# Bitcoin-Wildlife-Sanctuary/recursive-stwo

Hardware: AMD Instinct MI355X
Metric: recursive proofs verified/sec (higher is better)
Workload: dtype u32 (M31 modular integers)

## Files before the change

### recursive-stwo_amd/csrc/field.hpp

```cpp
#pragma once
#include <hip/hip_runtime.h>
#include <stdint.h>

namespace rsv {

constexpr uint32_t P = 0x7fffffffu;

__device__ __forceinline__ uint32_t m_add(uint32_t a, uint32_t b) {
    uint32_t s = a + b;
    return min(s, s - P);
}
__device__ __forceinline__ uint32_t m_sub(uint32_t a, uint32_t b) {
    uint32_t d = a - b;
    return min(d, d + P);
}
__device__ __forceinline__ uint32_t m_neg(uint32_t a) { return m_sub(0u, a); }
__device__ __forceinline__ uint32_t m_dbl(uint32_t a) { return m_add(a, a); }
__device__ __forceinline__ uint32_t m_mul(uint32_t a, uint32_t b) {
    uint64_t p = (uint64_t)a * b;
    uint32_t s = ((uint32_t)p & P) + (uint32_t)(p >> 31);
    return min(s, s - P);
}
__device__ __forceinline__ uint32_t m_sqr(uint32_t a) { return m_mul(a, a); }
__device__ __forceinline__ uint32_t m_shl(uint32_t a, uint32_t k) {
    return ((a << k) & P) | (a >> (31u - k));
}
__device__ inline uint32_t m_inv(uint32_t a) {
    uint32_t t1 = a;
    uint32_t t2 = m_mul(m_sqr(t1), t1);
    uint32_t t4 = t2;
    for (int i = 0; i < 2; i++) t4 = m_sqr(t4);
    t4 = m_mul(t4, t2);
    uint32_t t8 = t4;
    for (int i = 0; i < 4; i++) t8 = m_sqr(t8);
    t8 = m_mul(t8, t4);
    uint32_t t16 = t8;
    for (int i = 0; i < 8; i++) t16 = m_sqr(t16);
    t16 = m_mul(t16, t8);
    uint32_t t24 = t16;
    for (int i = 0; i < 8; i++) t24 = m_sqr(t24);
    t24 = m_mul(t24, t8);
    uint32_t t28 = t24;
    for (int i = 0; i < 4; i++) t28 = m_sqr(t28);
    t28 = m_mul(t28, t4);
    uint32_t t29 = m_mul(m_sqr(t28), t1);
    return m_mul(m_sqr(m_sqr(t29)), t1);
}

struct CM31 {
    uint32_t a, b;
};
struct QM31 {
    CM31 a, b;
};

__device__ __forceinline__ CM31 c_mk(uint32_t a, uint32_t b) { return CM31{a, b}; }
__device__ __forceinline__ CM31 c_add(CM31 x, CM31 y) { return {m_add(x.a, y.a), m_add(x.b, y.b)}; }
__device__ __forceinline__ CM31 c_sub(CM31 x, CM31 y) { return {m_sub(x.a, y.a), m_sub(x.b, y.b)}; }
__device__ __forceinline__ CM31 c_neg(CM31 x) { return {m_neg(x.a), m_neg(x.b)}; }
__device__ __forceinline__ CM31 c_mul(CM31 x, CM31 y) {
    return {m_sub(m_mul(x.a, y.a), m_mul(x.b, y.b)), m_add(m_mul(x.a, y.b), m_mul(x.b, y.a))};
}
__device__ __forceinline__ CM31 c_mul_m(CM31 x, uint32_t k) { return {m_mul(x.a, k), m_mul(x.b, k)}; }
__device__ __forceinline__ CM31 c_mul_r(CM31 x) {
    return {m_sub(m_dbl(x.a), x.b), m_add(m_dbl(x.b), x.a)};
}
__device__ inline CM31 c_inv(CM31 x) {
    uint32_t n = m_inv(m_add(m_sqr(x.a), m_sqr(x.b)));
    return {m_mul(x.a, n), m_mul(m_neg(x.b), n)};
}

__device__ __forceinline__ QM31 q_mk(uint32_t a0, uint32_t a1, uint32_t b0, uint32_t b1) {
    return QM31{{a0, a1}, {b0, b1}};
}
__device__ __forceinline__ QM31 q_zero() { return q_mk(0, 0, 0, 0); }
__device__ __forceinline__ QM31 q_one() { return q_mk(1, 0, 0, 0); }
__device__ __forceinline__ QM31 q_from_m(uint32_t x) { return q_mk(x, 0, 0, 0); }
__device__ __forceinline__ QM31 q_add(QM31 x, QM31 y) { return {c_add(x.a, y.a), c_add(x.b, y.b)}; }
__device__ __forceinline__ QM31 q_sub(QM31 x, QM31 y) { return {c_sub(x.a, y.a), c_sub(x.b, y.b)}; }
__device__ __forceinline__ QM31 q_neg(QM31 x) { return {c_neg(x.a), c_neg(x.b)}; }
__device__ __forceinline__ QM31 q_dbl(QM31 x) { return q_add(x, x); }
__device__ __forceinline__ QM31 q_mul(QM31 x, QM31 y) {
    CM31 ac = c_mul(x.a, y.a), bd = c_mul(x.b, y.b);
    return {c_add(ac, c_mul_r(bd)), c_add(c_mul(x.a, y.b), c_mul(x.b, y.a))};
}
__device__ __forceinline__ QM31 q_mul_m(QM31 x, uint32_t k) { return {c_mul_m(x.a, k), c_mul_m(x.b, k)}; }
__device__ __forceinline__ QM31 q_mul_c(QM31 x, CM31 k) { return {c_mul(x.a, k), c_mul(x.b, k)}; }
__device__ inline QM31 q_inv(QM31 x) {
    CM31 den = c_inv(c_sub(c_mul(x.a, x.a), c_mul_r(c_mul(x.b, x.b))));
    return {c_mul(x.a, den), c_mul(c_neg(x.b), den)};
}
__device__ __forceinline__ bool q_eq(QM31 x, QM31 y) {
    return ((x.a.a ^ y.a.a) | (x.a.b ^ y.a.b) | (x.b.a ^ y.b.a) | (x.b.b ^ y.b.b)) == 0;
}
__device__ __forceinline__ QM31 q_mul_i(QM31 x) { return q_mk(m_neg(x.a.b), x.a.a, m_neg(x.b.b), x.b.a); }
__device__ __forceinline__ QM31 q_mul_u(QM31 x) { return {c_mul_r(x.b), x.a}; }
__device__ __forceinline__ QM31 q_combine_ef(QM31 v0, QM31 v1, QM31 v2, QM31 v3) {
    return q_add(q_add(v0, q_mul_i(v1)), q_add(q_mul_u(v2), q_mul_u(q_mul_i(v3))));
}

}
```

### recursive-stwo_amd/csrc/k_plan.hpp

```cpp
#pragma once
#include "verify_common.hpp"

namespace rsv {

struct PlanPtrs {
    PlanHdr* hdr;
    uint32_t* ent;
    uint32_t* fl;
    uint32_t G, maxM;
    const uint32_t* ids;
    uint32_t p0;
    __device__ uint32_t proof_of(uint32_t slot) const { return ids ? ids[slot] : p0 + slot; }
};

constexpr int MAX_FUSED = 16;
template <class Args>
struct Fused {
    uint32_t nb;
    uint32_t lds_proofs;
    uint32_t first_block[MAX_FUSED + 1];
    uint8_t y_of[32];
    Args a[MAX_FUSED];
};
constexpr size_t plan_lds_bytes(uint32_t proofs) { return (size_t)proofs * (32 * 2 * 8 + 3 * 32 * 4); }
// ... 189 lines not shown
    const bool live = livep && j < nq;
    ProofCtx* c = livep ? &ctxs[p] : nullptr;
    const uint32_t gbase = grp * G;
    for (uint32_t i = threadIdx.x; i < pb * 32u * 2u; i += BLOCK) (&F[0][0][0])[i] = 0ull;
    const uint32_t v0 = live ? (c->raw_q[j] & ((1u << M) - 1u)) : 0xFFFFFFFFu;
    raw[threadIdx.x] = v0;
    __syncthreads();
    if (live) {
        uint32_t rank = 0;
        for (uint32_t k = 0; k < nq; k++) {
            const uint32_t vk = raw[gbase + k];
            rank += (vk < v0 || (vk == v0 && k < j)) ? 1u : 0u;
        }
        sq[gbase + rank] = v0;
        sp[gbase + rank] = (uint8_t)j;
    }
    __syncthreads();
    uint32_t flags = 0;
    const uint32_t v = live ? sq[gbase + j] : 0u;
    if (live) {
        c->q[j] = v;
        c->qperm[j] = sp[gbase + j];
        if (j + 1 < nq && sq[gbase + j + 1] == v) flags |= 1u << R_DUP_QUERY;
        uint32_t lstart = 0;
        if (j > 0) {
            const uint32_t x = v ^ sq[gbase + j - 1];
            lstart = x ? M - (31u - (uint32_t)__clz((int)x)) : M + 1u;
        }
        for (uint32_t l = lstart; l <= M; l++) atomicOr(&F[grp][l][j >> 6], 1ull << (j & 63u));
    }
    __syncthreads();
    auto mask = [&](uint32_t l) { return M128{F[grp][l][0], F[grp][l][1]}; };
    uint32_t sizes[3] = {M, A == B ? A : umax(A, B), A == B ? 0u : umin(A, B)};
    const uint32_t n_sizes = A == B ? 2u : 3u;
    auto is_size = [&](uint32_t l) { return l == sizes[0] || l == sizes[1] || (n_sizes == 3 && l == sizes[2]); };
    if (live) {
        for (uint32_t l = j; l <= M; l += nq) {
            const M128 Fl = mask(l);
            const uint32_t nodes = m128_pop(Fl);
            uint32_t lacking = 0;
            if (l >= 1) lacking = 2u * m128_pop(mask(l - 1)) - nodes;
            tl[grp][l] = nodes | (lacking << 8);
            if (l < M) {
                const uint32_t both_total = m128_pop(m128_andn(mask(l + 1), Fl));
                const uint32_t nosib_total = l == 0 ? 1u : m128_pop(mask(l - 1)) - m128_pop(m128_andn(Fl, mask(l - 1)));
                tw[grp][l] = (is_size(l + 1) ? 0u : nodes - both_total) + (is_size(l) ? 2u * nosib_total : 0u);
            }
        }
    }
    __syncthreads();
    PlanHdr* h = livep ? &pl.hdr[slot] : nullptr;
    if (live && j == 0) {
        uint32_t suffix = 0;
        h->lvl[M + 1] = 0;
        for (uint32_t l = M; l >= 1; l--) {
            suffix += (tl[grp][l] >> 8) & 0xFFu;
            h->lvl[l] = tl[grp][l] | (suffix << 16);
        }
        h->lvl[0] = 1u | (suffix << 16);
        uint32_t W = 0;
        for (uint32_t l = M; l-- > 0;) {
            wsum[grp][l] = W;
            h->wf[l + 1] = (uint16_t)W;
            W += tw[grp][l];
        }
        h->wf[0] = (uint16_t)W;
        h->wf_total = (uint16_t)umin(W, 0xFFFFu);
        c->n_sizes = n_sizes;
        c->sizes[0] = sizes[0]; c->sizes[1] = sizes[1]; c->sizes[2] = n_sizes == 3 ? sizes[2] : 0u;
        uint32_t base = 0;
        for (uint32_t g = 0; g < n_sizes; g++) {
            c->fw_base[g] = base;
            base += (tl[grp][sizes[g]] >> 8) & 0xFFu;
        }
        if (base != m->first.wit_n) flags |= (1u << R_FRI_FIRST) | F_RESCAN;
    }
    __syncthreads();
    if (live) {
        uint32_t* ent = pl.ent + (size_t)slot * (pl.maxM + 1) * G;
        uint32_t* fl = pl.fl + (size_t)slot * 2 * G;
        ent[j] = 0xFFu << 16;
        for (uint32_t l = 1; l <= M; l++) {
            const M128 Fl = mask(l), Fp = mask(l - 1);
            const uint32_t s = m128_last_le(Fp, j);
            const uint32_t e = m128_first_gt(Fp, j, nq) - 1u;
            const uint32_t Ns = m128_popbelow(Fl, s + 1), Ne = m128_popbelow(Fl, e + 1), Nj = m128_popbelow(Fl, j + 1);
            const bool both = Ne - Ns == 1u;
            const bool right = both && Nj - Ns == 1u;
            const uint32_t second = both ? m128_first_gt(Fl, s, nq) : 0u;
            const uint32_t sib = both ? (right ? second - 1u : second) : 0xFFu;
            const uint32_t lack_before = 2u * m128_popbelow(Fp, s) - m128_popbelow(Fl, s);
            ent[l * G + j] = (Nj - 1u) | (lack_before << 8) | (sib << 16);
        }
        for (uint32_t d = 0; d + 1 < n_sizes; d++) {
            const uint32_t l = sizes[1 + d];
            if (l >= M) continue;
            const M128 Fl = mask(l), Fc = mask(l + 1);
            const uint32_t f = m128_last_le(Fl, j), e = m128_first_gt(Fl, j, nq) - 1u;
            const bool has_both = m128_popbelow(Fc, e + 1) - m128_popbelow(Fc, f + 1) == 1u;
            const bool child_data = is_size(l + 1);
            const bool lack = !child_data && !has_both;
            bool sib_present = false;
            uint32_t nosib_before = 0;
            if (l >= 1) {
                const M128 Fp = mask(l - 1);
                const uint32_t s = m128_last_le(Fp, j), pe = m128_first_gt(Fp, j, nq) - 1u;
                sib_present = m128_popbelow(Fl, pe + 1) - m128_popbelow(Fl, s + 1) == 1u;
                nosib_before = m128_popbelow(Fp, s) - m128_popbelow(m128_andn(Fl, Fp), s);
            }
            const uint32_t nodes_before = m128_popbelow(Fl, f), both_before = m128_popbelow(m128_andn(Fc, Fl), f);
            const uint32_t base = wsum[grp][l] + (child_data ? 0u : nodes_before - both_before) + 2u * nosib_before;
            const bool odd = (v >> (M - l)) & 1u;
            uint32_t w_self = 0xFFFFu, w_sib = 0xFFFFu;
            if (odd) {
                if (!sib_present) w_sib = base;
                if (lack) w_self = base + (sib_present ? 0u : 2u);
            } else {
                if (lack) w_self = base;
                if (!sib_present) w_sib = base + (lack ? 1u : 0u);
            }
            fl[d * G + j] = (w_self & 0xFFFFu) | (w_sib << 16);
        }
    }
    if (flags) atomicOr(&c->flags, flags);
}

constexpr uint32_t TR_WORDS = 40 + 4 * (MAX_INNER + 1) + MAXQ;
__global__ __launch_bounds__(256) void k_export_transcript(uint32_t n, const ProofMeta* __restrict__ metas,
                                                            const ProofCtx* __restrict__ ctxs, uint32_t* __restrict__ out) {
    const size_t gid = (size_t)blockIdx.x * blockDim.x + threadIdx.x;
    if (gid >= (size_t)n * TR_WORDS) return;
    const uint32_t p = (uint32_t)(gid / TR_WORDS), k = (uint32_t)(gid % TR_WORDS);
    const ProofMeta& m = metas[p];
    const ProofCtx& c = ctxs[p];
    uint32_t v = 0;
    if (m.reason != R_OK || (c.flags & (1u << R_PARSE))) v = k == 0 ? (uint32_t)R_PARSE : 0u;
    else if (k == 0) v = (c.flags & (1u << R_POW)) ? (uint32_t)R_POW : (uint32_t)R_OK;
    else if (k == 1) v = m.n_inner + 1;
    else if (k == 2) v = m.nq;
    else if (k == 3) v = m.M;
    else if (k < 8) v = c.z[k - 4];
    else if (k < 12) v = c.alpha[k - 8];
    else if (k < 16) v = c.rc[k - 12];
    else if (k < 20) v = c.oods_t[k - 16];
    else if (k < 24) v = c.oods_x[k - 20];
    else if (k < 28) v = c.oods_y[k - 24];
    else if (k < 32) v = c.after[k - 28];
    else if (k < 40) v = c.pow_digest[k - 32];
    else if (k < 40 + 4 * (MAX_INNER + 1)) { uint32_t a = (k - 40) >> 2; v = a <= m.n_inner ? c.fri_alpha[a][(k - 40) & 3] : 0u; }
    else { uint32_t q = k - (40 + 4 * (MAX_INNER + 1)); v = q < m.nq ? c.raw_q[q] : 0u; }
    out[gid] = v;
}

__global__ __launch_bounds__(64) void k_qconst(const uint8_t* __restrict__ blob, const uint64_t* __restrict__ offsets,
                                               uint32_t n, const ProofMeta* __restrict__ metas,
                                               ProofCtx* __restrict__ ctxs) {
    const uint32_t p = blockIdx.x * blockDim.x + threadIdx.x;
    if (p >= n) return;
    const ProofMeta& m = metas[p];
    if (m.reason != R_OK) return;
    ProofCtx& c = ctxs[p];
    const uint32_t* w = reinterpret_cast<const uint32_t*>(blob + offsets[p]);
    const uint32_t M = m.M, A = m.A, B = m.B;
    uint32_t sizes[3] = {M, A == B ? A : umax(A, B), A == B ? 0u : umin(A, B)};
    const uint32_t n_sizes = A == B ? 2u : 3u;
    QM31 after = ldq(c.after);
    {
        QM31 ak = q_mk(0, 0, m_neg(2), 0);
#pragma unroll 1
        for (int k = 0; k < N_APOW; k++) { stq(c.apow[k], ak); ak = q_mul(ak, after); }
    }
    QM31 ox = ldq(c.oods_x), oy = ldq(c.oods_y);
    for (uint32_t g = 0; g < n_sizes; g++) {
        uint32_t l = sizes[g];
        uint32_t comp_log = (l == A) ? m.lp : m.lq;
        CPoint step = cp_gen_mul(1u << (31u - comp_log));
        step.y = m_neg(step.y);
        QM31 sx = q_sub(q_mul_m(ox, step.x), q_mul_m(oy, step.y));
        QM31 sy = q_add(q_mul_m(ox, step.y), q_mul_m(oy, step.x));
        uint32_t k_run = 0, n_batches = (l == M) ? 1u : 2u;
        for (uint32_t bi = 0; bi < n_batches; bi++) {
            QM31 px = bi ? sx : ox, py = bi ? sy : oy;
            QM31 sa = q_zero(), sb = q_zero();
            for (int t = 0; t < 4; t++) {
                uint32_t c0, c1;
                if (l == M) { if (t != 3) continue; c0 = 0; c1 = 8; }
                else {
                    if (t == 3) continue;
                    c0 = (l == A) ? 0u : plonk_cols(t);
                    c1 = (l == B) ? tree_cols(t) : plonk_cols(t);
                }
                for (uint32_t col = c0; col < c1; col++) {
                    uint32_t ns = n_samples_of(t, (int)col);
                    if (bi == 1 && ns != 2) continue;
                    int si = sample_index(t, (int)col, bi == 1 ? 0 : (int)ns - 1);
                    QM31 v = ldq(w + SAMPLES.off[si]);
                    QM31 ak = ldq(c.apow[k_run++]);
                    sa = q_add(sa, q_mul_c(ak, v.b));
                    sb = q_add(sb, q_mul_c(ak, c_sub(c_mul(v.a, py.b), c_mul(v.b, py.a))));
                }
            }
            QBatch& qb = c.batch[g][bi];
            stq(qb.sa, sa); stq(qb.sb, sb);
            qb.prx[0] = px.a.a; qb.prx[1] = px.a.b; qb.pix[0] = px.b.a; qb.pix[1] = px.b.b;
            qb.pry[0] = py.a.a; qb.pry[1] = py.a.b; qb.piy[0] = py.b.a; qb.piy[1] = py.b.b;
        }
        c.n_batches[g] = n_batches;
    }
}

__host__ __device__ constexpr int sample_index_c(int t, int col, int s) {
    return t == 0 ? S_T0 + col : t == 1 ? S_T1 + col : t == 3 ? S_T3 + col
         : S_T2 + (col < 4 ? col : col < 8 ? 4 + 2 * (col - 4) + s : col < 12 ? 12 + (col - 8) : 16 + 2 * (col - 12) + s);
}
struct QTab {
    uint16_t n[4];
    uint8_t si[4][N_APOW];
    uint8_t batch[4][N_APOW];
};
__host__ __device__ constexpr QTab make_qtab() {
    QTab q{};
    for (int kind = 0; kind < 4; kind++) {
        int k = 0;
        const int n_batches = kind == 0 ? 1 : 2;
        for (int bi = 0; bi < n_batches; bi++)
            for (int t = 0; t < 4; t++) {
                int c0 = 0, c1 = 0;
                if (kind == 0) { if (t != 3) continue; c0 = 0; c1 = 8; }
                else {
                    if (t == 3) continue;
                    c0 = (kind == 1 || kind == 3) ? 0 : (int)plonk_cols(t);
                    c1 = (kind == 2 || kind == 3) ? (int)tree_cols(t) : (int)plonk_cols(t);
                }
                for (int col = c0; col < c1; col++) {
                    const int ns = (int)n_samples_of(t, col);
                    if (bi == 1 && ns != 2) continue;
                    q.si[kind][k] = (uint8_t)sample_index_c(t, col, bi == 1 ? 0 : ns - 1);
                    q.batch[kind][k] = (uint8_t)bi;
                    k++;
                }
            }
        q.n[kind] = (uint16_t)k;
    }
    return q;
}
__constant__ QTab QTAB = make_qtab();
static_assert(make_qtab().n[3] <= N_APOW && make_qtab().n[3] == 134 && make_qtab().n[0] == 8, "alpha powers kept for the quotient numerators");

__global__ __launch_bounds__(256) void k_qconst_row(const uint8_t* __restrict__ blob, const uint64_t* __restrict__ offsets,
                                                    uint32_t n, const ProofMeta* __restrict__ metas,
                                                    ProofCtx* __restrict__ ctxs) {
    qconst_row_body(blockIdx.x, blob, offsets, n & 0x7FFFFFFFu, metas, ctxs, (n >> 31) != 0u);
}
__device__ void qconst_row_body(uint32_t block, const uint8_t* __restrict__ blob, const uint64_t* __restrict__ offsets, uint32_t n,
                                const ProofMeta* __restrict__ metas, ProofCtx* __restrict__ ctxs, bool four) {
    const uint32_t i = threadIdx.x & 15u, row = four ? (threadIdx.x >> 4) & 3u : 0u;
    const uint32_t p = (block * blockDim.x + threadIdx.x) >> (four ? 6 : 4);
    if (p >= n) return;
    const ProofMeta& m = metas[p];
    if (m.reason != R_OK) return;
    ProofCtx& c = ctxs[p];
    const uint32_t* w = reinterpret_cast<const uint32_t*>(blob + offsets[p]);
    const uint32_t M = m.M, A = m.A, B = m.B;
    const uint32_t sizes[3] = {M, A == B ? A : umax(A, B), A == B ? 0u : umin(A, B)};
    const uint32_t n_sizes = A == B ? 2u : 3u;
    auto sel = [](bool cnd, QM31 a, QM31 b) {
        return q_mk(cnd ? a.a.a : b.a.a, cnd ? a.a.b : b.a.b, cnd ? a.b.a : b.b.a, cnd ? a.b.b : b.b.b);
    };
    auto sum16 = [](QM31 x) { return q_mk(sum_row(x.a.a), sum_row(x.a.b), sum_row(x.b.a), sum_row(x.b.b)); };
    const QM31 after = ldq(c.after), one = q_one();
    const QM31 a2 = q_mul(after, after), a4 = q_mul(a2, a2), a8 = q_mul(a4, a4), a16 = q_mul(a8, a8);
    QM31 start = sel(i & 1u, after, one);
    start = q_mul(start, sel(i & 2u, a2, one));
    start = q_mul(start, sel(i & 4u, a4, one));
    start = q_mul(start, sel(i & 8u, a8, one));
    start = q_mul(start, q_mk(0, 0, m_neg(2), 0));
    if (!four || row == 3u) {
        QM31 cur = start;
#pragma unroll 1
        for (uint32_t k = i; k < (uint32_t)N_APOW; k += 16u) { stq(c.apow[k], cur); cur = q_mul(cur, a16); }
        if (four) return;
    }
    if (four && row >= n_sizes) return;
    const QM31 ox = ldq(c.oods_x), oy = ldq(c.oods_y);
    for (uint32_t g = four ? row : 0u; g < (four ? row + 1u : n_sizes); g++) {
        const uint32_t l = sizes[g];
        const uint32_t kind = l == M ? 0u : (A == B ? 3u : (l == A ? 1u : 2u));
        const uint32_t comp_log = (l == A) ? m.lp : m.lq;
        CPoint step = {GEN_POW.x[31u - comp_log], GEN_POW.y[31u - comp_log]};
        step.y = m_neg(step.y);
        const QM31 sx = q_sub(q_mul_m(ox, step.x), q_mul_m(oy, step.y));
        const QM31 sy = q_add(q_mul_m(ox, step.y), q_mul_m(oy, step.x));
        QM31 sa0 = q_zero(), sb0 = q_zero(), sa1 = q_zero(), sb1 = q_zero(), cur = start;
        const uint32_t cnt = QTAB.n[kind];
#pragma unroll 1
        for (uint32_t k0 = 0; k0 < cnt; k0 += 16u) {
            const uint32_t k = k0 + i;
            if (k < cnt) {
                const bool b1 = QTAB.batch[kind][k] != 0;
                const QM31 v = ldq(w + SAMPLES.off[QTAB.si[kind][k]]);
                const QM31 py = b1 ? sy : oy;
                const QM31 ta = q_mul_c(cur, v.b);
                const QM31 tb = q_mul_c(cur, c_sub(c_mul(v.a, py.b), c_mul(v.b, py.a)));
                sa0 = sel(b1, sa0, q_add(sa0, ta)); sb0 = sel(b1, sb0, q_add(sb0, tb));
                sa1 = sel(b1, q_add(sa1, ta), sa1); sb1 = sel(b1, q_add(sb1, tb), sb1);
            }
            cur = q_mul(cur, a16);
        }
        sa0 = sum16(sa0); sb0 = sum16(sb0); sa1 = sum16(sa1); sb1 = sum16(sb1);
        if (i == 0) {
            const uint32_t n_batches = (l == M) ? 1u : 2u;
            for (uint32_t bi = 0; bi < n_batches; bi++) {
                QBatch& qb = c.batch[g][bi];
                const QM31 px = bi ? sx : ox, py = bi ? sy : oy;
                stq(qb.sa, bi ? sa1 : sa0); stq(qb.sb, bi ? sb1 : sb0);
                qb.prx[0] = px.a.a; qb.prx[1] = px.a.b; qb.pix[0] = px.b.a; qb.pix[1] = px.b.b;
                qb.pry[0] = py.a.a; qb.pry[1] = py.a.b; qb.piy[0] = py.b.a; qb.piy[1] = py.b.b;
            }
            c.n_batches[g] = n_batches;
        }
    }
}

}
```

### recursive-stwo_amd/csrc/k_query.hpp

```cpp
#pragma once
#include "k_plan.hpp"

namespace rsv {

struct QueryArgs {
    const uint8_t* blob;
    const uint64_t* offsets;
    uint32_t n;
    const ProofMeta* metas;
    ProofCtx* ctxs;
    PlanPtrs pl;
    uint32_t* leafv;
    uint32_t maxInner;
    uint32_t* folded_out;
    uint32_t* qv_out;
    uint32_t qv_stride;
};

__device__ __forceinline__ uint32_t ent_rb(uint32_t e) { return e & 0xFFu; }
__device__ __forceinline__ uint32_t ent_lb(uint32_t e) { return (e >> 8) & 0xFFu; }
__device__ __forceinline__ uint32_t ent_sib(uint32_t e) { return (e >> 16) & 0xFFu; }
__device__ __forceinline__ uint32_t lvl_nd(uint32_t v) { return v & 0xFFu; }
__device__ __forceinline__ uint32_t lvl_tl(uint32_t v) { return (v >> 8) & 0xFFu; }
__device__ __forceinline__ uint32_t lvl_s(uint32_t v) { return v >> 16; }

__device__ inline QM31 fold_pair(QM31 self, QM31 sib, bool odd, uint32_t inv_coord, QM31 alpha) {
    QM31 l = odd ? sib : self, r = odd ? self : sib;
    return q_add(q_add(l, r), q_mul(q_mul_m(q_sub(l, r), inv_coord), alpha));
}

__device__ __forceinline__ QM31 line_eval(const uint32_t* __restrict__ cf, uint32_t log_n, uint32_t n, uint32_t x, uint32_t hi0 = 0,
                                          uint32_t hi_step = 1) {
    uint32_t r[16];
#pragma unroll
    for (int j = 0; j < 16; j++) { r[15 - j] = x; x = m_sub(m_dbl(m_sqr(x)), 1u); }
    const uint32_t s = (16u - log_n) & 15u;
#pragma unroll
    for (int st = 8; st >= 1; st >>= 1) {
        const bool on = (s & (uint32_t)st) != 0;
#pragma unroll
        for (int t = 0; t < 16; t++) {
            const uint32_t from = t + st < 16 ? r[t + st] : 1u;
            r[t] = on ? from : r[t];
        }
    }
    const uint32_t nlo = log_n < 4 ? log_n : 4u;
    uint32_t wl[16];
#pragma unroll
    for (int t = 0; t < 16; t++) wl[t] = 1u;
#pragma unroll
    for (int b = 0; b < 4; b++) {
        const uint32_t db = (uint32_t)b < nlo ? r[b] : 1u;
#pragma unroll
        for (int t = 0; t < 16; t++)
            if (t & (1 << b)) wl[t] = m_mul(wl[t], db);
    }
    QM31 acc = q_zero();
    const uint32_t n_hi = n >> nlo, n_lo = 1u << nlo;
#pragma unroll 1
    for (uint32_t hi = hi0; hi < n_hi; hi += hi_step) {
        uint32_t wh = 1u;
#pragma unroll
        for (int b = 0; b < 12; b++)
            if ((uint32_t)b + 4u < log_n && ((hi >> b) & 1u)) wh = m_mul(wh, r[b + 4]);
        QM31 inner = q_zero();
#pragma unroll
        for (int t = 0; t < 16; t++) {
            if ((uint32_t)t < n_lo) inner = q_add(inner, q_mul_m(ldq(cf + 4 * ((hi << nlo) + t)), wl[t]));
            if ((t & 3) == 3) __builtin_amdgcn_sched_barrier(0);
        }
        acc = q_add(acc, q_mul_m(inner, wh));
    }
    return acc;
}

__device__ __forceinline__ bool last_layer_ok(QM31 eval, QM31 folded) { return q_eq(eval, folded); }

template <int BLOCK, uint32_t QB, bool ROW = false>
__global__ __launch_bounds__(BLOCK) void k_query(Fused<QueryArgs> f) {
    constexpr int VB = ROW ? BLOCK / 16 : BLOCK;
    const uint32_t tid = ROW ? threadIdx.x >> 4 : threadIdx.x;
    const uint32_t part = ROW ? threadIdx.x & 15u : 0u;
    auto row_sum_q = [](QM31 v) { return q_mk(sum_row(v.a.a), sum_row(v.a.b), sum_row(v.b.a), sum_row(v.b.b)); };
    __shared__ uint32_t xq[VB][4];
    __shared__ uint32_t fst[3][4][VB];
    __shared__ uint32_t dps[3][2][VB];
    __builtin_amdgcn_s_setprio(3);
    RSV_FUSED_SELECT(f, a, bx);
    const uint32_t G = a.pl.G, per_block = VB / G;
    const uint32_t grp = tid / G, j = tid % G;
    const uint32_t slot = bx * per_block + grp;
    bool live = grp < per_block && slot < a.n;
    const uint32_t p = live ? a.pl.proof_of(slot) : 0u;
    const ProofMeta* m = live ? &a.metas[p] : nullptr;
    live = live && m->reason == R_OK && j < m->nq;
    ProofCtx* c = live ? &a.ctxs[p] : nullptr;
    const uint32_t* w = live ? reinterpret_cast<const uint32_t*>(a.blob + a.offsets[p]) : nullptr;
    const uint32_t* ent = live ? a.pl.ent + (size_t)slot * (a.pl.maxM + 1) * G : nullptr;
    const PlanHdr* h = live ? &a.pl.hdr[slot] : nullptr;
    uint32_t* leafv = live ? a.leafv + ((size_t)slot * (3 + a.maxInner)) * G * 8 : nullptr;
    const uint32_t gbase = grp * G;
    uint32_t flags = 0;
    uint32_t M = live ? m->M : 0, A = live ? m->A : 0, B = live ? m->B : 0;
    uint32_t qj = live ? c->q[j] : 0;
    uint32_t* qv = (live && a.qv_out) ? a.qv_out + ((size_t)slot * G + c->qperm[j]) * a.qv_stride : nullptr;
    uint32_t n_sizes = live ? c->n_sizes : 0;
    auto put_first = [&](uint32_t g, QM31 v) {
        fst[g][0][tid] = v.a.a; fst[g][1][tid] = v.a.b; fst[g][2][tid] = v.b.a; fst[g][3][tid] = v.b.b;
    };
    auto get_first = [&](uint32_t g) { return q_mk(fst[g][0][tid], fst[g][1][tid], fst[g][2][tid], fst[g][3][tid]); };
    if (live) {
        CPoint cur = domain_point(M, qj);
        uint32_t lvl = M;
        auto descend = [&](uint32_t g) {
            const uint32_t l = g < n_sizes ? c->sizes[g] : lvl;
            while (lvl > l) {
                const uint32_t pos = qj >> (M - lvl);
                uint32_t y2 = m_dbl(m_mul(cur.x, cur.y));
                cur.x = m_sub(m_dbl(m_sqr(cur.x)), 1u);
                cur.y = ((pos ^ (pos >> 1)) & 1u) ? m_neg(y2) : y2;
                lvl--;
            }
            dps[g][0][tid] = cur.x; dps[g][1][tid] = cur.y;
        };
        descend(0); descend(1); descend(2);
    }
    for (uint32_t g = 0; g < 3; g++) {
        QM31 answer = q_zero();
        uint32_t l = 0, pos = 0;
        bool on = live && g < n_sizes;
        uint32_t dpg_y = 0;
        if (on) {
            l = c->sizes[g];
            pos = qj >> (M - l);
            QM31 r0 = q_zero(), r1 = q_zero();
            uint32_t col = 0, dbl = 0;
            const uint32_t ncols_group = (l == M) ? 8u : ((l == A ? 30u : 0u) + (l == B ? 96u : 0u));
            for (int t = 0; t < 4; t++) {
                if ((l == M) != (t == 3)) continue;
                const uint32_t mx = (t == 3) ? M : umax(A, B);
                const uint32_t nc_leaf = (t == 3) ? 8u : ((A == mx ? plonk_cols(t) : 0u) + (B == mx ? poseidon_cols(t) : 0u));
                const uint32_t* qv = w + m->qv_off[t];
                const uint32_t qv_n = m->qv_n[t];
                for (int comp = 0; comp < 2; comp++) {
                    uint32_t cl = (t == 3) ? M : (comp == 0 ? A : B);
                    if (cl != l) continue;
                    uint32_t nc = (t == 3) ? (comp == 0 ? 8u : 0u) : (comp == 0 ? plonk_cols(t) : poseidon_cols(t));
                    if (nc == 0) continue;
                    uint32_t off;
                    if (cl == mx) off = ent_rb(ent[mx * G + j]) * nc_leaf + ((comp == 1 && A == B && t != 3) ? plonk_cols(t) : 0u);
                    else off = lvl_nd(h->lvl[mx]) * nc_leaf + ent_rb(ent[cl * G + j]) * nc;
                    bool inb = off + nc <= qv_n;
                    if (!inb) flags |= 1u << (R_MERKLE_T0 + t);
                    if constexpr (ROW) {
                        for (uint32_t k = part; k < nc; k += 16u) {
                            const uint32_t v = inb ? qv[off + k] : 0u;
                            r0 = q_add(r0, q_mul_m(ldq(c->apow[col + k]), v));
                            if (t == 2 && (k & 4u)) r1 = q_add(r1, q_mul_m(ldq(c->apow[ncols_group + dbl + 4u * (k >> 3) + (k & 3u)]), v));
                        }
                        col += nc;
                        if (t == 2) dbl += 4u * (nc >> 3) + ((nc & 7u) > 4u ? (nc & 7u) - 4u : 0u);
                    } else
                    for (uint32_t k0 = 0; k0 < nc; k0 += QB) {
                        const bool twice = t == 2 && (k0 & 4);
                        uint32_t vv[QB];
                        QM31 aa[QB];
#pragma unroll
                        for (uint32_t u = 0; u < QB; u++) {
                            const bool ok = k0 + u < nc;
                            vv[u] = (ok && inb) ? qv[off + k0 + u] : 0u;
                            aa[u] = ldq(c->apow[ok ? col + u : col]);
                        }
#pragma unroll
                        for (uint32_t u = 0; u < QB; u++) r0 = q_add(r0, q_mul_m(aa[u], vv[u]));
                        if (twice) {
#pragma unroll
                            for (uint32_t u = 0; u < QB; u++) aa[u] = ldq(c->apow[ncols_group + dbl + (k0 + u < nc ? u : 0u)]);
#pragma unroll
                            for (uint32_t u = 0; u < QB; u++) r1 = q_add(r1, q_mul_m(aa[u], vv[u]));
                        }
                        const uint32_t done = nc - k0 < QB ? nc - k0 : QB;
                        col += done;
                        if (twice) dbl += done;
                    }
                }
            }
            if constexpr (ROW) { r0 = row_sum_q(r0); r1 = row_sum_q(r1); }
            const CPoint dpg = {dps[g][0][tid], dps[g][1][tid]};
            dpg_y = dpg.y;
            for (uint32_t bi = 0; bi < c->n_batches[g]; bi++) {
                const QBatch& qb = c->batch[g][bi];
                CM31 prx = c_mk(qb.prx[0], qb.prx[1]), pix = c_mk(qb.pix[0], qb.pix[1]);
                CM31 pry = c_mk(qb.pry[0], qb.pry[1]), piy = c_mk(qb.piy[0], qb.piy[1]);
                CM31 den = c_sub(c_mul(c_sub(prx, c_mk(dpg.x, 0)), piy), c_mul(c_sub(pry, c_mk(dpg.y, 0)), pix));
                const CM31 inv_den = c_inv(den);
                __builtin_amdgcn_sched_barrier(0);
                QM31 num = q_sub(q_mul_c(bi ? r1 : r0, piy), q_add(q_mul_m(ldq(qb.sa), dpg.y), ldq(qb.sb)));
                answer = q_add(answer, q_mul_c(num, inv_den));
            }
        }
        stq(xq[tid], answer);
        __syncthreads();
        if (on) {
            uint32_t e = ent[l * G + j];
            QM31 sib;
            if (ent_sib(e) != 0xFFu) sib = ldq(xq[gbase + ent_sib(e)]);
            else {
                uint32_t wi = c->fw_base[g] + ent_lb(e);
                sib = wi < m->first.wit_n ? ldq(w + m->first.wit_off + 4 * wi) : q_zero();
                if ((sib.a.a >= P) | (sib.a.b >= P) | (sib.b.a >= P) | (sib.b.b >= P)) flags |= 1u << R_PARSE;
            }
            uint32_t* lv = leafv + ((size_t)g * G + j) * 8;
            stq(lv, answer); stq(lv + 4, sib);
            uint32_t by = (pos & 1u) ? m_neg(dpg_y) : dpg_y;
            const QM31 fg = fold_pair(answer, sib, pos & 1u, m_inv(by), ldq(c->fri_alpha[M - l]));
            put_first(g, fg);
            if (a.folded_out) stq(a.folded_out + (((size_t)slot * 3 + g) * G + c->qperm[j]) * 4, fg);
            if (qv) { stq(qv + 4 * g, answer); stq(qv + 12 + 4 * g, fg); }
        }
        __syncthreads();
    }
    QM31 folded = q_zero();
    uint32_t l = M;
    uint32_t X = live ? dps[0][0][tid] : 0u;
    for (uint32_t i = 0; i < a.maxInner; i++) {
        bool on = live && i < m->n_inner;
        if (on) {
            for (uint32_t g = 0; g < n_sizes; g++)
                if (c->sizes[g] == l) {
                    QM31 al = ldq(c->fri_alpha[i]);
                    folded = q_add(q_mul(q_mul(al, al), folded), get_first(g));
                }
            l -= 1;
        }
        stq(xq[tid], folded);
        __syncthreads();
        if (on) {
            uint32_t pos = qj >> (M - l);
            uint32_t e = ent[l * G + j];
            const FriLayerRef& L = m->inner[i];
            QM31 sib;
            if (ent_sib(e) != 0xFFu) sib = ldq(xq[gbase + ent_sib(e)]);
            else {
                uint32_t wi = ent_lb(e);
                sib = wi < L.wit_n ? ldq(w + L.wit_off + 4 * wi) : q_zero();
                if ((sib.a.a >= P) | (sib.a.b >= P) | (sib.b.a >= P) | (sib.b.b >= P)) flags |= 1u << R_PARSE;
            }
            if (j == 0 && lvl_tl(h->lvl[l]) != L.wit_n) flags |= (1u << R_FRI_INNER) | F_RESCAN;
            uint32_t* lv = leafv + ((size_t)(3 + i) * G + j) * 8;
            stq(lv, folded); stq(lv + 4, sib);
            if (qv) stq(qv + 24 + 4 * i, folded);
            uint32_t xr = (i == 0) ? X : m_sub(m_dbl(m_sqr(X)), 1u);
            X = (pos & 1u) ? m_neg(xr) : xr;
            folded = fold_pair(folded, sib, pos & 1u, m_inv(X), ldq(c->fri_alpha[i + 1]));
        }
        __syncthreads();
    }
    if (live) {
        QM31 acc = line_eval(w + m->last_off, m->log_last, m->last_n, m_sub(m_dbl(m_sqr(X)), 1u), part, ROW ? 16u : 1u);
        if constexpr (ROW) acc = row_sum_q(acc);
        if (!last_layer_ok(acc, folded)) flags |= 1u << R_FRI_LAST;
        if (qv) { stq(qv + 24 + 4 * a.maxInner, folded); stq(qv + 28 + 4 * a.maxInner, acc); }
    }
    if (flags) atomicOr(&c->flags, flags);
}

__global__ __launch_bounds__(256) void k_field_op(int op, const uint32_t* __restrict__ a, const uint32_t* __restrict__ b,
                                                   uint32_t* __restrict__ out, size_t n) {
    const size_t i = (size_t)blockIdx.x * blockDim.x + threadIdx.x;
    if (i >= n) return;
    QM31 x = ldq(a + 4 * i), y = b ? ldq(b + 4 * i) : q_zero(), r = q_zero();
    switch (op) {
        case 0: r = q_add(x, y); break;
        case 1: r = q_sub(x, y); break;
        case 2: r = q_mul(x, y); break;
        case 3: r = q_inv(x); break;
        case 4: r = q_mk(m_mul(x.a.a, y.a.a), 0, 0, 0); break;
        case 5: r = q_mk(m_inv(x.a.a), 0, 0, 0); break;
        case 6: { CM31 c = c_mul(x.a, y.a); r = q_mk(c.a, c.b, 0, 0); } break;
        case 7: { CM31 c = c_inv(x.a); r = q_mk(c.a, c.b, 0, 0); } break;
        case 8: r = q_mul_i(x); break;
        case 9: r = q_mul_u(x); break;
        case 10: {
            QM31 acc = q_one(), base = x;
            for (uint32_t e = y.a.a; e; e >>= 1) { if (e & 1u) acc = q_mul(acc, base); base = q_mul(base, base); }
            r = acc;
        } break;
        default: break;
    }
    stq(out + 4 * i, r);
}

__global__ __launch_bounds__(256) void k_domain_points(uint32_t log_size, const uint32_t* __restrict__ q,
                                                        uint32_t* __restrict__ xy, size_t n) {
    const size_t i = (size_t)blockIdx.x * blockDim.x + threadIdx.x;
    if (i >= n) return;
    CPoint p = domain_point(log_size, q[i] & ((1u << log_size) - 1u));
    xy[2 * i] = p.x; xy[2 * i + 1] = p.y;
}

__global__ __launch_bounds__(256) void k_last_layer_check(const uint32_t* __restrict__ coeffs, uint32_t log_n,
                                                           const uint32_t* __restrict__ x, const uint32_t* __restrict__ folded,
                                                           uint8_t* __restrict__ ok, size_t n) {
    const size_t i = (size_t)blockIdx.x * blockDim.x + threadIdx.x;
    if (i >= n) return;
    ok[i] = last_layer_ok(line_eval(coeffs, log_n, 1u << log_n, x[i]), ldq(folded + 4 * i)) ? 1 : 0;
}

__global__ __launch_bounds__(256) void k_line_eval(const uint32_t* __restrict__ coeffs, uint32_t log_n,
                                                    const uint32_t* __restrict__ x, uint32_t* __restrict__ out, size_t n) {
    const size_t i = (size_t)blockIdx.x * blockDim.x + threadIdx.x;
    if (i >= n) return;
    stq(out + 4 * i, line_eval(coeffs, log_n, 1u << log_n, x[i]));
}

}
```

### recursive-stwo_amd/csrc/layout.hpp

```cpp
#pragma once
#include <stdint.h>

#if !defined(__HIPCC__) && !defined(__host__)
#define __host__
#define __device__
#endif

namespace rsv {

constexpr int MAXQ = 128;
constexpr int MAX_INNER = 28;
constexpr int MAX_LOG = 30;
constexpr int N_SAMPLES = 142;
constexpr int N_APOW = 136;

__host__ __device__ constexpr uint32_t plonk_cols(int t) { return t == 0 ? 10u : t == 1 ? 12u : t == 2 ? 8u : 0u; }
__host__ __device__ constexpr uint32_t poseidon_cols(int t) { return t == 0 ? 40u : t == 1 ? 48u : t == 2 ? 8u : 0u; }
__host__ __device__ constexpr uint32_t tree_cols(int t) { return t == 3 ? 8u : plonk_cols(t) + poseidon_cols(t); }
__host__ __device__ constexpr uint32_t n_samples_of(int t, int c) { return (t == 2 && (c & 4)) ? 2u : 1u; }

constexpr uint32_t W_LP = 0, W_LQ = 1, W_PLONK_SUM = 2, W_POSEIDON_SUM = 6, W_POW_BITS = 10, W_BLOWUP = 11,
                   W_LOG_LAST = 12, W_NQ = 13, W_NCOMMIT = 15, W_COMMIT0 = 17, W_NTREES = 49;

struct SampleTable {
    uint16_t off[N_SAMPLES];
    uint16_t col_prefix[134];
    uint16_t tree_prefix[4];
    uint16_t end;
    uint16_t pre_of[N_SAMPLES];
    uint8_t cnt_of[N_SAMPLES];
};
__host__ __device__ constexpr SampleTable make_sample_table() {
    SampleTable t{};
    uint32_t pos = W_NTREES + 2, k = 0, c_all = 0;
    for (int tr = 0; tr < 4; tr++) {
        t.tree_prefix[tr] = (uint16_t)pos;
        pos += 2;
        for (uint32_t c = 0; c < tree_cols(tr); c++) {
            t.col_prefix[c_all++] = (uint16_t)pos;
            t.pre_of[k] = (uint16_t)pos;
            t.cnt_of[k] = (uint8_t)n_samples_of(tr, (int)c);
            pos += 2;
            for (uint32_t s = 0; s < n_samples_of(tr, (int)c); s++) {
                t.off[k++] = (uint16_t)pos;
                pos += 4;
            }
        }
    }
    t.end = (uint16_t)pos;
    return t;
}
constexpr int S_T0 = 0, S_T1 = 50, S_T2 = 110, S_T3 = 134;

struct FriLayerRef {
    uint32_t wit_off, wit_n;
    uint32_t hash_off, hash_n;
    uint32_t commit_off;
};

struct ProofMeta {
    uint32_t reason;
    uint32_t n_words;
    uint32_t lp, lq, pow_bits, blowup, log_last, nq, n_inner, A, B, M;
    uint32_t hw_off[4], hw_n[4];
    uint32_t qv_off[4], qv_n[4];
    uint32_t nonce_off;
    FriLayerRef first;
    FriLayerRef inner[MAX_INNER];
    uint32_t last_off, last_n;
};


struct QBatch {
    uint32_t sa[4], sb[4];
    uint32_t prx[2], pix[2], pry[2], piy[2];
};

constexpr uint32_t F_RESCAN = 1u << 30;
constexpr uint32_t F_REASON_MASK = (1u << 13) - 1u;

struct ProofCtx {
    uint32_t flags;
    uint32_t flow_on;
    uint32_t front_over;
    uint32_t n_sizes;
    uint32_t sizes[3];
    uint32_t fw_base[3];
    uint32_t z[4], alpha[4], rc[4], oods_t[4], oods_x[4], oods_y[4], after[4];
    uint32_t pow_digest[8];
    uint32_t fri_alpha[MAX_INNER + 1][4];
    uint32_t raw_q[MAXQ];
    uint32_t q[MAXQ];
    uint8_t qperm[MAXQ];
    QBatch batch[3][2];
    uint32_t n_batches[3];
    uint32_t apow[N_APOW][4];
};

__host__ __device__ constexpr uint32_t flow_chunks(uint32_t n_cols) { return (n_cols + 7u) / 8u; }
__host__ __device__ constexpr uint32_t flow_transcript_len(uint32_t nq, uint32_t n_inner, uint32_t last_n) {
    return 82u + 2u * (1u + n_inner) + (last_n + 1u) / 2u + 1u + (nq + 3u) / 4u;
}
__host__ __device__ constexpr uint32_t flow_trace_path_len(int t, uint32_t A, uint32_t B, uint32_t M) {
    const uint32_t mx = t == 3 ? M : (A > B ? A : B);
    const uint32_t nc_leaf = t == 3 ? 8u : ((A == mx ? plonk_cols(t) : 0u) + (B == mx ? poseidon_cols(t) : 0u));
    const uint32_t nc_lower = (t == 3 || A == B) ? 0u : (A < B ? plonk_cols(t) : poseidon_cols(t));
    return flow_chunks(nc_leaf) + 1u + mx + (nc_lower ? flow_chunks(nc_lower) + 1u : 0u);
}
__host__ __device__ constexpr uint32_t flow_pair_path_len(uint32_t s, uint32_t A, uint32_t B, uint32_t M) {
    return s == 0 ? 4u + M + 4u * (A == B ? 1u : 2u) : 4u + (M - s);
}
__host__ __device__ constexpr uint32_t flow_trace_base(int t, uint32_t nq, uint32_t n_inner, uint32_t last_n, uint32_t A, uint32_t B,
                                                       uint32_t M) {
    uint32_t at = flow_transcript_len(nq, n_inner, last_n);
    for (int k = 0; k < t; k++) at += nq * flow_trace_path_len(k, A, B, M);
    return at;
}
__host__ __device__ constexpr uint32_t flow_pair_base(uint32_t s, uint32_t nq, uint32_t n_inner, uint32_t last_n, uint32_t A, uint32_t B,
                                                      uint32_t M) {
    uint32_t at = flow_trace_base(4, nq, n_inner, last_n, A, B, M);
    for (uint32_t k = 0; k < s; k++) at += nq * flow_pair_path_len(k, A, B, M);
    return at;
}
__host__ __device__ constexpr uint32_t flow_total(uint32_t nq, uint32_t n_inner, uint32_t last_n, uint32_t A, uint32_t B, uint32_t M) {
    return flow_pair_base(1u + n_inner, nq, n_inner, last_n, A, B, M);
}
constexpr uint32_t FLOW_WORDS = 32;

struct PlanHdr {
    uint32_t lvl[MAX_LOG + 2];
    uint16_t wf[MAX_LOG + 2];
    uint16_t wf_total, pad;
};

enum WitnessOp : uint32_t {
    W_CONST, W_ADD, W_MUL, W_MULC, W_COPY, W_INV, W_INV0, W_QINV, W_CINV, W_COORD, W_BIT, W_FLOW, W_WORD, W_WORD4,
    W_FRI_COMMIT, W_LAST_POLY, W_NONCE, W_TRACE_COL, W_FRI_COL, W_N_OPS
};

}
```

Before: 2.264 million.

## Batch field inversions, lazily reduce dot products, precompute squared FRI alphas

Several arithmetic restructurings in the query kernel. Per-query field inversions (quotient denominators, fold y-inverses, inner-layer x-inverses) are now computed with one Montgomery batch inversion, with results kept in shared memory and a parking buffer. Column dot products now accumulate unreduced 64-bit partial sums through v_mad_u64_u32 with a lazy fold instead of reducing after every multiply. The polynomial evaluation computes its weights from precomputed pairwise products, and squared FRI alphas are computed once per group in k_qconst. This removes many modular inversions and reductions, but adds register pressure, inline assembly and extra shared or global traffic.

```diff
diff --git a/recursive-stwo_amd/csrc/field.hpp b/recursive-stwo_amd/csrc/field.hpp
--- a/recursive-stwo_amd/csrc/field.hpp
+++ b/recursive-stwo_amd/csrc/field.hpp
@@ -90,6 +90,47 @@
     CM31 den = c_inv(c_sub(c_mul(x.a, x.a), c_mul_r(c_mul(x.b, x.b))));
     return {c_mul(x.a, den), c_mul(c_neg(x.b), den)};
 }
+constexpr int LAZY_TERMS = 2;
+struct QAcc {
+    uint64_t aa, ab, ba, bb;
+};
+__device__ __forceinline__ uint64_t l_mul(uint32_t a, uint32_t v) {
+    uint64_t d, carry;
+    asm("v_mad_u64_u32 %0, %1, %2, %3, 0" : "=v"(d), "=s"(carry) : "v"(a), "v"(v));
+    return d;
+}
+__device__ __forceinline__ uint64_t l_mad(uint32_t a, uint32_t v, uint64_t s) {
+    uint64_t d, carry;
+    asm("v_mad_u64_u32 %0, %1, %2, %3, %4" : "=v"(d), "=s"(carry) : "v"(a), "v"(v), "v"(s));
+    return d;
+}
+__device__ __forceinline__ uint64_t l_fold(uint64_t s, uint64_t T) {
+    uint64_t d, e, carry;
+    asm("v_mad_u64_u32 %0, %1, %2, 2, %3" : "=v"(d), "=s"(carry) : "v"((uint32_t)(s >> 32)), "v"(T));
+    asm("v_mad_u64_u32 %0, %1, %2, 1, %3" : "=v"(e), "=s"(carry) : "v"((uint32_t)s), "v"(d));
+    return e;
+}
+__device__ __forceinline__ uint32_t l_red32(uint64_t T) {
+    const uint64_t f = (uint64_t)(uint32_t)(T >> 32) * 2u + (uint32_t)T;
+    return ((uint32_t)f & P) + (uint32_t)(f >> 31);
+}
+__device__ __forceinline__ uint32_t l_canon(uint64_t T) {
+    const uint32_t r = l_red32(T);
+    return min(r, r - P);
+}
+__device__ __forceinline__ QAcc qa_zero() { return QAcc{0, 0, 0, 0}; }
+__device__ __forceinline__ void qa_mad2(QAcc& T, QM31 x, uint32_t v, QM31 y, uint32_t w) {
+    static_assert(LAZY_TERMS == 2, "two terms per fold");
+    T.aa = l_fold(l_mad(y.a.a, w, l_mul(x.a.a, v)), T.aa); T.ab = l_fold(l_mad(y.a.b, w, l_mul(x.a.b, v)), T.ab);
+    T.ba = l_fold(l_mad(y.b.a, w, l_mul(x.b.a, v)), T.ba); T.bb = l_fold(l_mad(y.b.b, w, l_mul(x.b.b, v)), T.bb);
+}
+__device__ __forceinline__ void qa_mad1(QAcc& T, QM31 x, uint32_t v) {
+    T.aa = l_fold(l_mul(x.a.a, v), T.aa); T.ab = l_fold(l_mul(x.a.b, v), T.ab);
+    T.ba = l_fold(l_mul(x.b.a, v), T.ba); T.bb = l_fold(l_mul(x.b.b, v), T.bb);
+}
+__device__ __forceinline__ QM31 qa_canon(const QAcc& T) { return q_mk(l_canon(T.aa), l_canon(T.ab), l_canon(T.ba), l_canon(T.bb)); }
+__device__ __forceinline__ QM31 qa_red32(const QAcc& T) { return q_mk(l_red32(T.aa), l_red32(T.ab), l_red32(T.ba), l_red32(T.bb)); }
+
 __device__ __forceinline__ bool q_eq(QM31 x, QM31 y) {
     return ((x.a.a ^ y.a.a) | (x.a.b ^ y.a.b) | (x.b.a ^ y.b.a) | (x.b.b ^ y.b.b)) == 0;
 }
diff --git a/recursive-stwo_amd/csrc/k_plan.hpp b/recursive-stwo_amd/csrc/k_plan.hpp
--- a/recursive-stwo_amd/csrc/k_plan.hpp
+++ b/recursive-stwo_amd/csrc/k_plan.hpp
@@ -365,6 +365,12 @@
     out[gid] = v;
 }
 
+__device__ __forceinline__ void store_alpha_sq(ProofCtx& c, const ProofMeta& m, uint32_t g, uint32_t l) {
+    const uint32_t i = m.M - l;
+    if (i > m.n_inner) return;
+    const QM31 al = ldq(c.fri_alpha[i]);
+    stq(c.fri_alpha_sq[g], q_mul(al, al));
+}
 __global__ __launch_bounds__(64) void k_qconst(const uint8_t* __restrict__ blob, const uint64_t* __restrict__ offsets,
                                                uint32_t n, const ProofMeta* __restrict__ metas,
                                                ProofCtx* __restrict__ ctxs) {
@@ -419,6 +425,7 @@
             qb.pry[0] = py.a.a; qb.pry[1] = py.a.b; qb.piy[0] = py.b.a; qb.piy[1] = py.b.b;
         }
         c.n_batches[g] = n_batches;
+        store_alpha_sq(c, m, g, l);
     }
 }
 
@@ -531,8 +538,9 @@
                 qb.pry[0] = py.a.a; qb.pry[1] = py.a.b; qb.piy[0] = py.b.a; qb.piy[1] = py.b.b;
             }
             c.n_batches[g] = n_batches;
-        }
-    }
-}
-
-}
+            store_alpha_sq(c, m, g, l);
+        }
+    }
+}
+
+}
diff --git a/recursive-stwo_amd/csrc/k_query.hpp b/recursive-stwo_amd/csrc/k_query.hpp
--- a/recursive-stwo_amd/csrc/k_query.hpp
+++ b/recursive-stwo_amd/csrc/k_query.hpp
@@ -55,29 +55,39 @@
         for (int t = 0; t < 16; t++)
             if (t & (1 << b)) wl[t] = m_mul(wl[t], db);
     }
-    QM31 acc = q_zero();
+    const uint32_t f4 = 4u < log_n ? r[4] : 1u, f5 = 5u < log_n ? r[5] : 1u, f6 = 6u < log_n ? r[6] : 1u, f7 = 7u < log_n ? r[7] : 1u;
+    const uint32_t f45 = m_mul(f4, f5), f67 = m_mul(f6, f7);
+    QAcc acc = qa_zero();
     const uint32_t n_hi = n >> nlo, n_lo = 1u << nlo;
 #pragma unroll 1
     for (uint32_t hi = hi0; hi < n_hi; hi += hi_step) {
-        uint32_t wh = 1u;
-#pragma unroll
-        for (int b = 0; b < 12; b++)
-            if ((uint32_t)b + 4u < log_n && ((hi >> b) & 1u)) wh = m_mul(wh, r[b + 4]);
-        QM31 inner = q_zero();
-#pragma unroll
-        for (int t = 0; t < 16; t++) {
-            if ((uint32_t)t < n_lo) inner = q_add(inner, q_mul_m(ldq(cf + 4 * ((hi << nlo) + t)), wl[t]));
-            if ((t & 3) == 3) __builtin_amdgcn_sched_barrier(0);
-        }
-        acc = q_add(acc, q_mul_m(inner, wh));
-    }
-    return acc;
+        const uint32_t wa = (hi & 2u) ? ((hi & 1u) ? f45 : f5) : ((hi & 1u) ? f4 : 1u);
+        const uint32_t wb = (hi & 8u) ? ((hi & 4u) ? f67 : f7) : ((hi & 4u) ? f6 : 1u);
+        uint32_t wh = m_mul(wa, wb);
+        if (hi >> 4) {
+#pragma unroll
+            for (int b = 4; b < 12; b++)
+                if ((uint32_t)b + 4u < log_n && ((hi >> b) & 1u)) wh = m_mul(wh, r[b + 4]);
+        }
+        QAcc inner = qa_zero();
+#pragma unroll
+        for (int t = 0; t < 16; t += 2) {
+            if ((uint32_t)t < n_lo) {
+                const bool two = (uint32_t)t + 1u < n_lo;
+                qa_mad2(inner, ldq(cf + 4 * ((hi << nlo) + t)), wl[t], ldq(cf + 4 * ((hi << nlo) + (two ? t + 1 : t))), two ? wl[t + 1] : 0u);
+            }
+            if ((t & 3) == 2) __builtin_amdgcn_sched_barrier(0);
+        }
+        qa_mad1(acc, qa_red32(inner), wh);
+    }
+    return qa_canon(acc);
 }
 
 __device__ __forceinline__ bool last_layer_ok(QM31 eval, QM31 folded) { return q_eq(eval, folded); }
 
 template <int BLOCK, uint32_t QB, bool ROW = false>
 __global__ __launch_bounds__(BLOCK) void k_query(Fused<QueryArgs> f) {
+    static_assert(QB % LAZY_TERMS == 0, "a batch of loads is a whole number of folds");
     constexpr int VB = ROW ? BLOCK / 16 : BLOCK;
     const uint32_t tid = ROW ? threadIdx.x >> 4 : threadIdx.x;
     const uint32_t part = ROW ? threadIdx.x & 15u : 0u;
@@ -85,6 +95,7 @@
     __shared__ uint32_t xq[VB][4];
     __shared__ uint32_t fst[3][4][VB];
     __shared__ uint32_t dps[3][2][VB];
+    constexpr uint32_t XIV = 8;
     __builtin_amdgcn_s_setprio(3);
     RSV_FUSED_SELECT(f, a, bx);
     const uint32_t G = a.pl.G, per_block = VB / G;
@@ -125,15 +136,57 @@
         };
         descend(0); descend(1); descend(2);
     }
+    const uint32_t n_parked = live ? (m->n_inner < a.maxInner ? m->n_inner : a.maxInner) : 0u;
+    uint32_t* park = n_parked ? leafv + ((size_t)(3 + n_parked - 1) * G + j) * 8 : nullptr;
+    auto quotient_den = [&](const QBatch& qb, uint32_t x, uint32_t y) {
+        CM31 prx = c_mk(qb.prx[0], qb.prx[1]), pix = c_mk(qb.pix[0], qb.pix[1]);
+        CM31 pry = c_mk(qb.pry[0], qb.pry[1]), piy = c_mk(qb.piy[0], qb.piy[1]);
+        return c_sub(c_mul(c_sub(prx, c_mk(x, 0)), piy), c_mul(c_sub(pry, c_mk(y, 0)), pix));
+    };
+    if (live) {
+        constexpr int NS = 9 + (int)XIV;
+        uint32_t v[NS];
+#pragma unroll
+        for (int g = 0; g < 3; g++) {
+            const uint32_t x = dps[g][0][tid], y = dps[g][1][tid];
+#pragma unroll
+            for (int bi = 0; bi < 2; bi++) {
+                v[3 * g + bi] = 0u;
+                if ((uint32_t)g < n_sizes && (uint32_t)bi < c->n_batches[g]) {
+                    const CM31 den = quotient_den(c->batch[g][bi], x, y);
+                    v[3 * g + bi] = m_add(m_sqr(den.a), m_sqr(den.b));
+                }
+            }
+            v[3 * g + 2] = (uint32_t)g < n_sizes ? y : 0u;
+        }
+        uint32_t xr = dps[0][0][tid];
+#pragma unroll
+        for (int i = 0; i < (int)XIV; i++) {
+            v[9 + i] = (uint32_t)i < m->n_inner ? xr : 0u;
+            xr = m_sub(m_dbl(m_sqr(xr)), 1u);
+        }
+        uint32_t run = 1u, pre[XIV];
+#pragma unroll
+        for (int k = 0; k < NS; k++) {
+            if (k < 9) fst[k / 3][k % 3][tid] = run; else pre[k - 9] = run;
+            run = m_mul(run, v[k] ? v[k] : 1u);
+        }
+        run = m_inv(run);
+#pragma unroll
+        for (int k = NS - 1; k >= 0; k--) {
+            if (k < 9) fst[k / 3][k % 3][tid] = v[k] ? m_mul(run, fst[k / 3][k % 3][tid]) : 0u;
+            else if ((uint32_t)(k - 9) < n_parked) park[k - 9] = v[k] ? m_mul(run, pre[k - 9]) : 0u;
+            run = m_mul(run, v[k] ? v[k] : 1u);
+        }
+    }
     for (uint32_t g = 0; g < 3; g++) {
         QM31 answer = q_zero();
         uint32_t l = 0, pos = 0;
         bool on = live && g < n_sizes;
-        uint32_t dpg_y = 0;
         if (on) {
             l = c->sizes[g];
             pos = qj >> (M - l);
-            QM31 r0 = q_zero(), r1 = q_zero();
+            QAcc s0 = qa_zero(), s1 = qa_zero();
             uint32_t col = 0, dbl = 0;
             const uint32_t ncols_group = (l == M) ? 8u : ((l == A ? 30u : 0u) + (l == B ? 96u : 0u));
             for (int t = 0; t < 4; t++) {
@@ -153,10 +206,14 @@
                     bool inb = off + nc <= qv_n;
                     if (!inb) flags |= 1u << (R_MERKLE_T0 + t);
                     if constexpr (ROW) {
-                        for (uint32_t k = part; k < nc; k += 16u) {
-                            const uint32_t v = inb ? qv[off + k] : 0u;
-                            r0 = q_add(r0, q_mul_m(ldq(c->apow[col + k]), v));
-                            if (t == 2 && (k & 4u)) r1 = q_add(r1, q_mul_m(ldq(c->apow[ncols_group + dbl + 4u * (k >> 3) + (k & 3u)]), v));
+                        static_assert(LAZY_TERMS == 2, "the row form takes two columns per pass");
+                        for (uint32_t k = part; k < nc; k += 32u) {
+                            const uint32_t k1 = k + 16u < nc ? k + 16u : k;
+                            const uint32_t v = inb ? qv[off + k] : 0u, v1 = (inb && k + 16u < nc) ? qv[off + k1] : 0u;
+                            qa_mad2(s0, ldq(c->apow[col + k]), v, ldq(c->apow[col + k1]), v1);
+                            if (t == 2 && (k & 4u))
+                                qa_mad2(s1, ldq(c->apow[ncols_group + dbl + 4u * (k >> 3) + (k & 3u)]), v,
+                                        ldq(c->apow[ncols_group + dbl + 4u * (k1 >> 3) + (k1 & 3u)]), v1);
                         }
                         col += nc;
                         if (t == 2) dbl += 4u * (nc >> 3) + ((nc & 7u) > 4u ? (nc & 7u) - 4u : 0u);
@@ -172,12 +229,12 @@
                             aa[u] = ldq(c->apow[ok ? col + u : col]);
                         }
 #pragma unroll
-                        for (uint32_t u = 0; u < QB; u++) r0 = q_add(r0, q_mul_m(aa[u], vv[u]));
+                        for (uint32_t u = 0; u < QB; u += 2) qa_mad2(s0, aa[u], vv[u], aa[u + 1], vv[u + 1]);
                         if (twice) {
 #pragma unroll
                             for (uint32_t u = 0; u < QB; u++) aa[u] = ldq(c->apow[ncols_group + dbl + (k0 + u < nc ? u : 0u)]);
 #pragma unroll
-                            for (uint32_t u = 0; u < QB; u++) r1 = q_add(r1, q_mul_m(aa[u], vv[u]));
+                            for (uint32_t u = 0; u < QB; u += 2) qa_mad2(s1, aa[u], vv[u], aa[u + 1], vv[u + 1]);
                         }
                         const uint32_t done = nc - k0 < QB ? nc - k0 : QB;
                         col += done;
@@ -185,15 +242,15 @@
                     }
                 }
             }
+            QM31 r0 = qa_canon(s0), r1 = qa_canon(s1);
             if constexpr (ROW) { r0 = row_sum_q(r0); r1 = row_sum_q(r1); }
             const CPoint dpg = {dps[g][0][tid], dps[g][1][tid]};
-            dpg_y = dpg.y;
             for (uint32_t bi = 0; bi < c->n_batches[g]; bi++) {
                 const QBatch& qb = c->batch[g][bi];
-                CM31 prx = c_mk(qb.prx[0], qb.prx[1]), pix = c_mk(qb.pix[0], qb.pix[1]);
-                CM31 pry = c_mk(qb.pry[0], qb.pry[1]), piy = c_mk(qb.piy[0], qb.piy[1]);
-                CM31 den = c_sub(c_mul(c_sub(prx, c_mk(dpg.x, 0)), piy), c_mul(c_sub(pry, c_mk(dpg.y, 0)), pix));
-                const CM31 inv_den = c_inv(den);
+                const CM31 piy = c_mk(qb.piy[0], qb.piy[1]);
+                const CM31 den = quotient_den(qb, dpg.x, dpg.y);
+                const uint32_t inv_norm = fst[g][bi][tid];
+                const CM31 inv_den = {m_mul(den.a, inv_norm), m_mul(m_neg(den.b), inv_norm)};
                 __builtin_amdgcn_sched_barrier(0);
                 QM31 num = q_sub(q_mul_c(bi ? r1 : r0, piy), q_add(q_mul_m(ldq(qb.sa), dpg.y), ldq(qb.sb)));
                 answer = q_add(answer, q_mul_c(num, inv_den));
@@ -212,8 +269,8 @@
             }
             uint32_t* lv = leafv + ((size_t)g * G + j) * 8;
             stq(lv, answer); stq(lv + 4, sib);
-            uint32_t by = (pos & 1u) ? m_neg(dpg_y) : dpg_y;
-            const QM31 fg = fold_pair(answer, sib, pos & 1u, m_inv(by), ldq(c->fri_alpha[M - l]));
+            const uint32_t inv_y = fst[g][2][tid];
+            const QM31 fg = fold_pair(answer, sib, pos & 1u, (pos & 1u) ? m_neg(inv_y) : inv_y, ldq(c->fri_alpha[M - l]));
             put_first(g, fg);
             if (a.folded_out) stq(a.folded_out + (((size_t)slot * 3 + g) * G + c->qperm[j]) * 4, fg);
             if (qv) { stq(qv + 4 * g, answer); stq(qv + 12 + 4 * g, fg); }
@@ -227,10 +284,8 @@
         bool on = live && i < m->n_inner;
         if (on) {
             for (uint32_t g = 0; g < n_sizes; g++)
-                if (c->sizes[g] == l) {
-                    QM31 al = ldq(c->fri_alpha[i]);
-                    folded = q_add(q_mul(q_mul(al, al), folded), get_first(g));
-                }
+                if (c->sizes[g] == l)
+                    folded = q_add(q_mul(ldq(c->fri_alpha_sq[g]), folded), get_first(g));
             l -= 1;
         }
         stq(xq[tid], folded);
@@ -248,11 +303,13 @@
             }
             if (j == 0 && lvl_tl(h->lvl[l]) != L.wit_n) flags |= (1u << R_FRI_INNER) | F_RESCAN;
             uint32_t* lv = leafv + ((size_t)(3 + i) * G + j) * 8;
+            const uint32_t inv_x = i < XIV ? park[i] : 0u;
             stq(lv, folded); stq(lv + 4, sib);
             if (qv) stq(qv + 24 + 4 * i, folded);
             uint32_t xr = (i == 0) ? X : m_sub(m_dbl(m_sqr(X)), 1u);
             X = (pos & 1u) ? m_neg(xr) : xr;
-            folded = fold_pair(folded, sib, pos & 1u, m_inv(X), ldq(c->fri_alpha[i + 1]));
+            const uint32_t inv_xr = i < XIV ? inv_x : m_inv(xr);
+            folded = fold_pair(folded, sib, pos & 1u, (pos & 1u) ? m_neg(inv_xr) : inv_xr, ldq(c->fri_alpha[i + 1]));
         }
         __syncthreads();
     }
diff --git a/recursive-stwo_amd/csrc/layout.hpp b/recursive-stwo_amd/csrc/layout.hpp
--- a/recursive-stwo_amd/csrc/layout.hpp
+++ b/recursive-stwo_amd/csrc/layout.hpp
@@ -95,6 +95,7 @@
     QBatch batch[3][2];
     uint32_t n_batches[3];
     uint32_t apow[N_APOW][4];
+    uint32_t fri_alpha_sq[3][4];
 };
 
 __host__ __device__ constexpr uint32_t flow_chunks(uint32_t n_cols) { return (n_cols + 7u) / 8u; }
```

Result: no change. 2.286 million, median of 6 (+0.9%).
